# t0m1ab/alphazero

Measured on AMD Instinct MI355X. Metric: self-play games/sec (whole node), Othello 8x8 @100 sims/move, higher is better.
Workload: dtype f32; 1 GPU; BASELINE configs[1] literal: Othello 8x8, 4096 concurrent games/GPU, 100 sims/move, 1 MI355X; concurrent_games_per_gpu=4096, sims_per_move=100, parallelism=game-sharded x1, dense_layers=float32 fma chains on the f32-input MFMA

## Files before the change

### alphazero_amd/csrc/az_net.hip

```cpp
#include <math.h>
#include <stdlib.h>
#include <string.h>

#include <map>
#include <string>
#include <vector>

#include "az_device.h"
#include <hip/hip_ext.h>
#include "az_host.h"

typedef float f32x4 __attribute__((ext_vector_type(4)));
#define MFMA(a, b, c) __builtin_amdgcn_mfma_f32_16x16x4f32((a), (b), (c), 0, 0, 0)
typedef float f32x16 __attribute__((ext_vector_type(16)));
typedef float f32x2 __attribute__((ext_vector_type(2)));
#define MFMA32(a, b, c) __builtin_amdgcn_mfma_f32_32x32x2f32((a), (b), (c), 0, 0, 0)

#define NCH 32
#define PLANE_STRIDE(x) (((x) + 1) | 1)

#ifdef AZ_PROBE
__device__ unsigned long long az_probe_buf[8192 * 8];
#define STAMP(var) { __builtin_amdgcn_sched_barrier(0); var = __builtin_amdgcn_s_memtime(); asm volatile("s_waitcnt lgkmcnt(0)" ::: "memory"); __builtin_amdgcn_sched_barrier(0); }
#else
// ... 19 lines not shown
    const int m_lane = lane & 15, kq = lane >> 4;
    int abase[MT];
    unsigned vmask[MT];
#pragma unroll
    for (int mt = 0; mt < MT; ++mt) {
        int p = 16 * mt + m_lane;
        p = p < P_OUT ? p : P_OUT - 1;
        const int y = p / W_OUT, x = p % W_OUT;
        abase[mt] = kq * IN_PS + y * IN_W + x - PAD * (IN_W + 1);
        unsigned vm = 0;
#pragma unroll
        for (int t = 0; t < 9; ++t) {
            int iy = y + t / 3 - PAD, ix = x + t % 3 - PAD;
            vm |= (unsigned)(iy >= 0 && iy < H_OUT + 2 - 2 * PAD && ix >= 0 && ix < W_OUT + 2 - 2 * PAD) << t;
        }
        vmask[mt] = vm;
    }
    const float *wl = wf + 4 * lane;
    float bfr[2][16];
#pragma unroll
    for (int q = 0; q < 4; ++q) {
        const f32x4 v = *reinterpret_cast<const f32x4 *>(wl + q * 256);
        bfr[0][4 * q] = v[0]; bfr[0][4 * q + 1] = v[1]; bfr[0][4 * q + 2] = v[2]; bfr[0][4 * q + 3] = v[3];
    }
    const float bv0 = bias[m_lane], bv1 = bias[16 + m_lane];
#pragma unroll
    for (int mt = 0; mt < MT; ++mt) {
        acc[mt][0] = (f32x4){bv0, bv0, bv0, bv0};
        acc[mt][1] = (f32x4){bv1, bv1, bv1, bv1};
    }
    float ar[A_RING][MT];
#define CONV_LOAD(c, mt) in_lds[abase[mt] + ((c) / 8 / 3) * IN_W + ((c) / 8 % 3) + 4 * ((c) % 8) * IN_PS]
#pragma unroll
    for (int c = 0; c < A_RING; ++c)
#pragma unroll
        for (int mt = 0; mt < MT; ++mt) ar[c][mt] = CONV_LOAD(c, mt);
#pragma unroll
    for (int c = 0; c < 72; ++c) {
        const int tap = c / 8, j = c % 8;
        if (j == 0 && tap < 8) {
#pragma unroll
            for (int q = 0; q < 4; ++q) {
                const f32x4 v = *reinterpret_cast<const f32x4 *>(wl + ((tap + 1) * 4 + q) * 256);
                bfr[(tap + 1) & 1][4 * q] = v[0]; bfr[(tap + 1) & 1][4 * q + 1] = v[1];
                bfr[(tap + 1) & 1][4 * q + 2] = v[2]; bfr[(tap + 1) & 1][4 * q + 3] = v[3];
            }
        }
        float ac[MT];
#pragma unroll
        for (int mt = 0; mt < MT; ++mt) {
            float v = ar[c % A_RING][mt];
            if (PAD) v = ((vmask[mt] >> tap) & 1u) ? v : 0.0f;
            ac[mt] = v;
        }
        if (c + A_RING < 72) {
#pragma unroll
            for (int mt = 0; mt < MT; ++mt) ar[c % A_RING][mt] = CONV_LOAD(c + A_RING, mt);
        }
        __builtin_amdgcn_sched_barrier(0);
#pragma unroll
        for (int mt = 0; mt < MT; ++mt) {
            acc[mt][0] = MFMA(ac[mt], bfr[tap & 1][2 * j + 0], acc[mt][0]);
            acc[mt][1] = MFMA(ac[mt], bfr[tap & 1][2 * j + 1], acc[mt][1]);
        }
        __builtin_amdgcn_sched_barrier(0);
    }
#undef CONV_LOAD
}

template <int P_OUT, int OUT_PS, int MT>
AZ_D void store_relu_lds(float *out, int lane, const f32x4 (&acc)[MT][2]) {
#pragma unroll
    for (int mt = 0; mt < MT; ++mt)
#pragma unroll
        for (int nt = 0; nt < 2; ++nt)
#pragma unroll
            for (int r = 0; r < 4; ++r) {
                int m = 16 * mt + (lane >> 4) * 4 + r;
                float v = acc[mt][nt][r];
                if (m < P_OUT) out[(nt * 16 + (lane & 15)) * OUT_PS + m] = v > 0.0f ? v : 0.0f;
            }
}

template <int CH, int CW, int PS, int RING>
AZ_D void conv2_wino(float *act, const float4 *wu4, const float *__restrict__ bias, int lane) {
    constexpr int TW = (CW + 1) / 2, NTL = ((CH + 1) / 2) * TW, P1 = CH * CW;
    static_assert(NTL <= 16 && PS > P1, "one 16-row tile of 2x2 output tiles per board; a zero slot behind every plane");
    const int m = lane & 15, kq = lane >> 4;
    const int t = m < NTL ? m : NTL - 1;
    const int ty = t / TW, tx = t % TW;
    const float4 *ul = wu4 + lane;
    float cu[2][4][2], cw_[2][4][2];
    float yo[2][4][2][2];
#pragma unroll
    for (int p = 0; p < 2; ++p) {
        int off[12];
#pragma unroll
        for (int a = 0; a < 3; ++a)
#pragma unroll
            for (int b = 0; b < 4; ++b) {
                const int iy = 2 * ty - 1 + a + p, ix = 2 * tx - 1 + b;
                off[a * 4 + b] = kq * PS + ((iy >= 0 && iy < CH && ix >= 0 && ix < CW) ? iy * CW + ix : P1);
            }
        f32x4 acc[8][2];
#pragma unroll
        for (int f = 0; f < 8; ++f) { acc[f][0] = (f32x4){0.0f, 0.0f, 0.0f, 0.0f}; acc[f][1] = (f32x4){0.0f, 0.0f, 0.0f, 0.0f}; }
        float4 ub[RING][4];
#pragma unroll
        for (int jj = 0; jj < RING - 1; ++jj)
#pragma unroll
            for (int q = 0; q < 4; ++q) ub[jj][q] = ul[(size_t)((p * 8 + jj) * 4 + q) * 64];
        float d[12];
#pragma unroll
        for (int e = 0; e < 12; ++e) d[e] = act[off[e]];
#pragma unroll
        for (int j = 0; j < 8; ++j) {
            float dn[12];
            if (j + RING - 1 < 8) {
#pragma unroll
                for (int q = 0; q < 4; ++q) ub[(j + RING - 1) % RING][q] = ul[(size_t)((p * 8 + j + RING - 1) * 4 + q) * 64];
            }
            if (j + 1 < 8) {
#pragma unroll
                for (int e = 0; e < 12; ++e) dn[e] = act[off[e] + 4 * (j + 1) * PS];
            }
            float T[2][4], V[8];
#pragma unroll
            for (int b = 0; b < 4; ++b) {
                if (p == 0) { T[0][b] = d[b] - d[8 + b]; T[1][b] = d[4 + b] + d[8 + b]; }
                else { T[0][b] = d[4 + b] - d[b]; T[1][b] = d[b] - d[8 + b]; }
            }
#pragma unroll
            for (int i = 0; i < 2; ++i) {
                V[4 * i + 0] = T[i][0] - T[i][2]; V[4 * i + 1] = T[i][1] + T[i][2];
                V[4 * i + 2] = T[i][2] - T[i][1]; V[4 * i + 3] = T[i][1] - T[i][3];
            }
            __builtin_amdgcn_sched_barrier(0);
#pragma unroll
            for (int f = 0; f < 8; ++f) {
                const float4 u = ub[j % RING][f >> 1];
                acc[f][0] = MFMA(V[f], (f & 1) ? u.z : u.x, acc[f][0]);
                acc[f][1] = MFMA(V[f], (f & 1) ? u.w : u.y, acc[f][1]);
            }
#pragma unroll
            for (int f = 0; f < 8; ++f) { asm volatile("" : "+a"(acc[f][0])); asm volatile("" : "+a"(acc[f][1])); }
            __builtin_amdgcn_sched_barrier(0);
            if (j + 1 < 8) {
#pragma unroll
                for (int e = 0; e < 12; ++e) d[e] = dn[e];
            }
        }
#pragma unroll
        for (int nt = 0; nt < 2; ++nt)
#pragma unroll
            for (int r = 0; r < 4; ++r) {
                float R[2][2];
#pragma unroll
                for (int i = 0; i < 2; ++i) {
                    R[i][0] = (acc[4 * i + 0][nt][r] + acc[4 * i + 1][nt][r]) + acc[4 * i + 2][nt][r];
                    R[i][1] = (acc[4 * i + 1][nt][r] - acc[4 * i + 2][nt][r]) - acc[4 * i + 3][nt][r];
                }
#pragma unroll
                for (int c = 0; c < 2; ++c) {
                    if (p == 0) { cu[nt][r][c] = R[0][c] + R[1][c]; cw_[nt][r][c] = R[1][c]; }
                    else { yo[nt][r][0][c] = cu[nt][r][c] + R[0][c]; yo[nt][r][1][c] = (cw_[nt][r][c] - R[0][c]) - R[1][c]; }
                }
            }
    }
    LDS_FENCE();
#pragma unroll
    for (int nt = 0; nt < 2; ++nt) {
        const float bv = bias[nt * 16 + m];
#pragma unroll
        for (int r = 0; r < 4; ++r) {
            const int tt = 4 * kq + r, y0 = 2 * (tt / TW), x0 = 2 * (tt % TW);
#pragma unroll
            for (int i = 0; i < 2; ++i)
#pragma unroll
                for (int c = 0; c < 2; ++c) {
                    const float v = yo[nt][r][i][c] + bv;
                    if (tt < NTL && y0 + i < CH && x0 + c < CW) act[(nt * 16 + m) * PS + (y0 + i) * CW + x0 + c] = v > 0.0f ? v : 0.0f;
                }
        }
    }
}

template <int CH, int CW, int PS, int OFF1>
AZ_D void conv2_wino32(float *act, const float2 *u2, const float *__restrict__ bias, int lane) {
    constexpr int TW = (CW + 1) / 2, NTL = ((CH + 1) / 2) * TW, P1 = CH * CW;
    static_assert(2 * NTL <= 32 && PS > P1, "the tiles of two boards fill one 32-row MFMA tile");
    const int m = lane & 31, kk = lane >> 5;
    const int mc = m < 2 * NTL ? m : 2 * NTL - 1;
    const int bd = mc / NTL, t = mc % NTL, ty = t / TW, tx = t % TW;
    int off[16];
#pragma unroll
    for (int a = 0; a < 4; ++a)
#pragma unroll
        for (int b = 0; b < 4; ++b) {
            const int iy = 2 * ty - 1 + a, ix = 2 * tx - 1 + b;
            off[a * 4 + b] = bd * OFF1 + kk * PS + ((iy >= 0 && iy < CH && ix >= 0 && ix < CW) ? iy * CW + ix : P1);
        }
    f32x16 acc[16];
#pragma unroll
    for (int f = 0; f < 16; ++f)
#pragma unroll
        for (int i = 0; i < 16; ++i) acc[f][i] = 0.0f;
    const float2 *ul = u2 + lane;
    float d[16], V[2][16];
#define DP(e) ((f32x2){d[e], d[(e) + 1]})
#define WINO32_STAGE1(q, Tl, Th)                              \
    {                                                         \
        if ((q) == 0) Tl[0] = DP(0) - DP(8);                  \
        if ((q) == 1) Th[0] = DP(2) - DP(10);                 \
        if ((q) == 2) Tl[1] = DP(4) + DP(8);                  \
        if ((q) == 3) Th[1] = DP(6) + DP(10);                 \
        if ((q) == 4) Tl[2] = DP(8) - DP(4);                  \
        if ((q) == 5) Th[2] = DP(10) - DP(6);                 \
        if ((q) == 6) Tl[3] = DP(4) - DP(12);                 \
        if ((q) == 7) Th[3] = DP(6) - DP(14);                 \
    }
#define WINO32_STAGE2(i, c, Tl, Th, Vout)                                                          \
    {                                                                                              \
        if ((c) == 0) { const f32x2 v03 = Tl[i] - Th[i]; Vout[4 * (i) + 0] = v03.x; Vout[4 * (i) + 3] = v03.y; } \
        if ((c) == 1) Vout[4 * (i) + 1] = Tl[i].y + Th[i].x;                                       \
        if ((c) == 2) Vout[4 * (i) + 2] = Th[i].x - Tl[i].y;                                       \
    }
#define WINO32_FENCE() { __builtin_amdgcn_sched_barrier(0); asm volatile("" ::: "memory"); __builtin_amdgcn_sched_barrier(0); }
#pragma unroll
    for (int e = 0; e < 16; ++e) d[e] = act[off[e]];
    float2 ub[2][16];
#pragma unroll
    for (int f = 0; f < 16; ++f) ub[0][f] = ul[f * 64];
    {
        f32x2 Tl[4], Th[4];
#pragma unroll
        for (int q = 0; q < 8; ++q) WINO32_STAGE1(q, Tl, Th)
#pragma unroll
        for (int i = 0; i < 4; ++i)
#pragma unroll
            for (int c = 0; c < 3; ++c) WINO32_STAGE2(i, c, Tl, Th, V[0])
    }
#pragma unroll
    for (int e = 0; e < 16; ++e) d[e] = act[off[e] + 2 * PS];
    WINO32_FENCE()
    constexpr int DORD[16] = {0, 1, 8, 9, 2, 3, 10, 11, 4, 5, 6, 7, 12, 13, 14, 15};
#pragma unroll
    for (int j = 0; j < 16; ++j) {
        f32x2 Tl[4], Th[4];
#pragma unroll
        for (int g = 0; g < 16; ++g) {
            if (j + 1 < 16) {
                if (g < 8) WINO32_STAGE1(g, Tl, Th)
                if (g >= 2 && g < 14) WINO32_STAGE2((g - 2) / 3, (g - 2) % 3, Tl, Th, V[(j + 1) & 1])
            }
            if (j + 2 < 16 && g >= 8) {
                const int e0 = DORD[2 * (g - 8)], e1 = DORD[2 * (g - 8) + 1];
                d[e0] = act[off[e0] + 2 * (j + 2) * PS];
                d[e1] = act[off[e1] + 2 * (j + 2) * PS];
            }
            if (j % 2 == 0 && j + 2 < 16) ub[(j / 2 + 1) & 1][g] = ul[((j / 2 + 1) * 16 + g) * 64];
            WINO32_FENCE()
            acc[g] = MFMA32(V[j & 1][g], (j % 2 == 0) ? ub[(j / 2) & 1][g].x : ub[(j / 2) & 1][g].y, acc[g]);
            asm volatile("" : "+a"(acc[g]));
            WINO32_FENCE()
// ... 120 lines not shown
#pragma unroll
    for (int i = 0; i < NA; ++i)
        if (i < nu) {
#pragma unroll
            for (int q = 0; q < 4; ++q) {
                const int r = 16 * (par + 2 * i) + (lane >> 4) * 4 + q;
                const float v = acc[i][q];
                if (r < rows) out[(r / P_OUT) * OUT_BS + (nt * 16 + (lane & 15)) * OUT_CS + r % P_OUT] = v > 0.0f ? v : 0.0f;
            }
        }
}

template <int CH, int CW, bool WINO>
__global__ __launch_bounds__(256, 2) void k_trunk(const float *__restrict__ in, int B, const int *__restrict__ dyn_count, TrunkParams tp, float *__restrict__ feat) {
    using G = TrunkGeom<CH, CW>;
    if (dyn_count) { int c = *dyn_count; B = c < B ? c : B; }
    extern __shared__ __attribute__((aligned(16))) float smem[];
    const int wave = threadIdx.x >> 6, lane = threadIdx.x & 63;
    const int b = blockIdx.x * 4 + wave;
    if (b >= B) return;
    float *inp = smem + wave * G::WAVE_FLOATS;
    float *act = inp + G::INP;
    for (int i = lane; i < G::INP; i += 64) inp[i] = 0.0f;
    if (WINO && lane < NCH) act[lane * G::PS + G::P1] = 0.0f;
    LDS_FENCE();
    for (int p = lane; p < G::P1; p += 64) inp[(p / CW + 1) * G::PW + (p % CW) + 1] = in[(size_t)b * G::P1 + p];
    LDS_FENCE();
    {
        f32x4 acc[G::MT2][2];
        const int m_lane = lane & 15, kq = lane >> 4;
        const float bv0 = tp.b1[m_lane], bv1 = tp.b1[16 + m_lane];
#pragma unroll
        for (int s = 0; s < 3; ++s) {
            int tap = 4 * s + kq;
            tap = tap < 9 ? tap : 8;
            const int toff = (tap / 3) * G::PW + tap % 3;
            const float b0 = tp.w1f[(s * 2 + 0) * 64 + lane], b1 = tp.w1f[(s * 2 + 1) * 64 + lane];
#pragma unroll
            for (int mt = 0; mt < G::MT2; ++mt) {
                int p = 16 * mt + m_lane;
                p = p < G::P1 ? p : G::P1 - 1;
                const float a = inp[(p / CW) * G::PW + (p % CW) + toff];
                if (s == 0) { acc[mt][0] = (f32x4){bv0, bv0, bv0, bv0}; acc[mt][1] = (f32x4){bv1, bv1, bv1, bv1}; }
                acc[mt][0] = MFMA(a, b0, acc[mt][0]);
                acc[mt][1] = MFMA(a, b1, acc[mt][1]);
            }
        }
        store_relu_lds<G::P1, G::PS, G::MT2>(act, lane, acc);
    }
    LDS_FENCE();
    if constexpr (WINO) {
        conv2_wino<CH, CW, G::PS, 3>(act, reinterpret_cast<const float4 *>(tp.wu), tp.cb[0], lane);
    } else {
        f32x4 acc[G::MT2][2];
        conv_mfma<G::P1, CW, CH, CW, G::PS, 1, G::MT2>(act, tp.wq[0], tp.cb[0], lane, acc);
        LDS_FENCE();
        store_relu_lds<G::P1, G::PS, G::MT2>(act, lane, acc);
    }
    LDS_FENCE();
    {
        f32x4 acc[G::MT3][2];
        conv_mfma<G::P3, G::W3, G::H3, CW, G::PS, 0, G::MT3>(act, tp.wq[1], tp.cb[1], lane, acc);
        LDS_FENCE();
        store_relu_lds<G::P3, G::PS, G::MT3>(act, lane, acc);
    }
    LDS_FENCE();
    {
        f32x4 acc[G::MT4][2];
        conv_mfma<G::P4, G::W4, G::H4, G::W3, G::PS, 0, G::MT4>(act, tp.wq[2], tp.cb[2], lane, acc);
        float *fo = feat + (size_t)b * (NCH * G::P4);
#pragma unroll
        for (int mt = 0; mt < G::MT4; ++mt)
#pragma unroll
            for (int nt = 0; nt < 2; ++nt)
#pragma unroll
                for (int r = 0; r < 4; ++r) {
                    int m = 16 * mt + (lane >> 4) * 4 + r;
                    float v = acc[mt][nt][r];
                    if (m < G::P4) fo[(nt * 16 + (lane & 15)) * G::P4 + m] = v > 0.0f ? v : 0.0f;
                }
    }
}

template <int CH, int CW>
__global__ __launch_bounds__(256, 2) void k_trunk_quad(const float *__restrict__ in, int B, const int *__restrict__ dyn_count, TrunkParams tp, float *__restrict__ feat) {
    using G = TrunkGeom<CH, CW>;
    if (dyn_count) { int c = *dyn_count; B = c < B ? c : B; }
    extern __shared__ __attribute__((aligned(16))) float smem[];
    const int wave = threadIdx.x >> 6, lane = threadIdx.x & 63;
    const int b = blockIdx.x * 4 + wave;
    if ((int)blockIdx.x * 4 >= B) return;
    const bool has = b < B;
    const int nb = B - (int)blockIdx.x * 4 < 4 ? B - (int)blockIdx.x * 4 : 4;
    const int nt = wave >> 1, par = (wave & 1) ^ (__builtin_popcount(blockIdx.x) & 1);
    float *inp = smem + wave * G::WAVE_FLOATS;
    float *act = inp + G::INP;
    float *act0 = smem + G::INP;
    if (has) {
        for (int i = lane; i < G::INP; i += 64) inp[i] = 0.0f;
        if (lane < NCH) act[lane * G::PS + G::P1] = 0.0f;
        LDS_FENCE();
        for (int p = lane; p < G::P1; p += 64) inp[(p / CW + 1) * G::PW + (p % CW) + 1] = in[(size_t)b * G::P1 + p];
        LDS_FENCE();
    }
    if (has) {
        f32x4 acc[G::MT2][2];
        const int m_lane = lane & 15, kq = lane >> 4;
        const float bv0 = tp.b1[m_lane], bv1 = tp.b1[16 + m_lane];
#pragma unroll
        for (int s = 0; s < 3; ++s) {
            int tap = 4 * s + kq;
            tap = tap < 9 ? tap : 8;
            const int toff = (tap / 3) * G::PW + tap % 3;
            const float b0 = tp.w1f[(s * 2 + 0) * 64 + lane], b1 = tp.w1f[(s * 2 + 1) * 64 + lane];
#pragma unroll
            for (int mt = 0; mt < G::MT2; ++mt) {
                int p = 16 * mt + m_lane;
                p = p < G::P1 ? p : G::P1 - 1;
                const float a = inp[(p / CW) * G::PW + (p % CW) + toff];
                if (s == 0) { acc[mt][0] = (f32x4){bv0, bv0, bv0, bv0}; acc[mt][1] = (f32x4){bv1, bv1, bv1, bv1}; }
                acc[mt][0] = MFMA(a, b0, acc[mt][0]);
                acc[mt][1] = MFMA(a, b1, acc[mt][1]);
            }
        }
        store_relu_lds<G::P1, G::PS, G::MT2>(act, lane, acc);
        LDS_FENCE();
    }
    if (has) {
        conv2_wino<CH, CW, G::PS, 3>(act, reinterpret_cast<const float4 *>(tp.wu), tp.cb[0], lane);
        LDS_FENCE();
    }
    __syncthreads();
    {
        f32x4 acc[((4 * G::P3 + 15) / 16 + 1) / 2];
        const int nu = conv_quad_deal<G::P3, G::W3, CW, G::PS, G::WAVE_FLOATS>(act0, tp.wq[1], tp.cb[1], lane, nt, par, nb * G::P3, acc);
        __syncthreads();
        store_quad_relu<G::P3, G::PS, G::WAVE_FLOATS>(act0, lane, nt, par, nu, nb * G::P3, acc);
    }
    __syncthreads();
    {
        f32x4 acc[((4 * G::P4 + 15) / 16 + 1) / 2];
        const int nu = conv_quad_deal<G::P4, G::W4, G::W3, G::PS, G::WAVE_FLOATS>(act0, tp.wq[2], tp.cb[2], lane, nt, par, nb * G::P4, acc);
        store_quad_relu<G::P4, G::P4, NCH * G::P4>(feat + (size_t)blockIdx.x * 4 * (NCH * G::P4), lane, nt, par, nu, nb * G::P4, acc);
    }
}

template <int P_OUT, int W_OUT, int H_OUT, int IN_W, int IN_PS, int PAD>
AZ_D f32x4 conv_tile(const float *in_lds, const float *__restrict__ wf, const float *__restrict__ bias, int lane, int mt, int nt) {
    const int m_lane = lane & 15, kq = lane >> 4;
    int p = 16 * mt + m_lane;
    p = p < P_OUT ? p : P_OUT - 1;
    const int y = p / W_OUT, x = p % W_OUT;
    const int abase = kq * IN_PS + y * IN_W + x - PAD * (IN_W + 1);
    unsigned vmask = 0;
#pragma unroll
    for (int t = 0; t < 9; ++t) {
        int iy = y + t / 3 - PAD, ix = x + t % 3 - PAD;
        vmask |= (unsigned)(iy >= 0 && iy < H_OUT + 2 - 2 * PAD && ix >= 0 && ix < W_OUT + 2 - 2 * PAD) << t;
    }
    const float *wl = wf + 4 * lane;
    float bfr[2][8];
#define TILE_BLOAD(tap_, buf_)                                                             \
    _Pragma("unroll") for (int q = 0; q < 4; ++q) {                                        \
        const f32x4 v = *reinterpret_cast<const f32x4 *>(wl + ((tap_) * 4 + q) * 256);     \
        bfr[buf_][2 * q] = nt ? v[1] : v[0];                                               \
        bfr[buf_][2 * q + 1] = nt ? v[3] : v[2];                                           \
    }
    TILE_BLOAD(0, 0)
    const float bv = bias[16 * nt + m_lane];
    f32x4 acc = (f32x4){bv, bv, bv, bv};
    float ar[A_RING];
#define TILE_LOAD(c) in_lds[abase + ((c) / 8 / 3) * IN_W + ((c) / 8 % 3) + 4 * ((c) % 8) * IN_PS]
#pragma unroll
    for (int c = 0; c < A_RING; ++c) ar[c] = TILE_LOAD(c);
#pragma unroll
    for (int c = 0; c < 72; ++c) {
        const int tap = c / 8, j = c % 8;
        if (j == 0 && tap < 8) { TILE_BLOAD(tap + 1, (tap + 1) & 1) }
        float v = ar[c % A_RING];
        if (PAD) v = ((vmask >> tap) & 1u) ? v : 0.0f;
        if (c + A_RING < 72) ar[c % A_RING] = TILE_LOAD(c + A_RING);
        __builtin_amdgcn_sched_barrier(0);
        acc = MFMA(v, bfr[tap & 1][j], acc);
        __builtin_amdgcn_sched_barrier(0);
    }
#undef TILE_LOAD
#undef TILE_BLOAD
    return acc;
}

template <int P_OUT, int OUT_PS>
AZ_D void store_tile_relu_lds(float *out, int lane, const f32x4 &acc, int mt, int nt) {
#pragma unroll
    for (int r = 0; r < 4; ++r) {
        const int m = 16 * mt + (lane >> 4) * 4 + r;
        const float v = acc[r];
        if (m < P_OUT) out[(nt * 16 + (lane & 15)) * OUT_PS + m] = v > 0.0f ? v : 0.0f;
    }
}

template <int CH, int CW, int PS>
AZ_D void conv2_wino_pass(const float *act, const float4 *wu4, int lane, int nt, int p, float (&R)[4][2][2]) {
    constexpr int TW = (CW + 1) / 2, NTL = ((CH + 1) / 2) * TW, P1 = CH * CW, RING = 3;
    const int m = lane & 15, kq = lane >> 4;
    const int t = m < NTL ? m : NTL - 1;
    const int ty = t / TW, tx = t % TW;
    const float4 *ul = wu4 + lane + (size_t)p * 8 * 4 * 64;
    int off[12];
#pragma unroll
    for (int a = 0; a < 3; ++a)
#pragma unroll
        for (int b = 0; b < 4; ++b) {
// ... 2388 lines not shown
            AZ_TRY(fold_launch(n, FOLD_BIAS, (float *)n->tp.cb[l - 1], NCH, "", 0, cn + ".bias", NCH, bnn, NCH, 0, 0, 0, st));
            AZ_TRY(fold_launch(n, FOLD_WP, (float *)n->tp.wp[l - 1], 9 * 16 * 64, cn + ".weight", wn, "", 0, bnn, NCH, 0, 0, 0, st));
            AZ_TRY(fold_launch(n, FOLD_WQ, (float *)n->tp.wq[l - 1], 9 * 16 * 64, cn + ".weight", wn, "", 0, bnn, NCH, 0, 0, 0, st));
            if (l == 1) AZ_TRY(fold_launch(n, FOLD_WINO, (float *)n->tp.wu, 2 * 8 * 4 * 64 * 4, cn + ".weight", wn, "", 0, bnn, NCH, 0, 0, 0, st));
            if (l == 1) AZ_TRY(fold_launch(n, FOLD_WINO32, (float *)n->tp.wu32, 4 * 16 * 64 * 4, cn + ".weight", wn, "", 0, bnn, NCH, 0, 0, 0, st));
        }
    }
    AZ_TRY(fold_launch(n, FOLD_DENSE_T, n->fc1w, n->FIN * n->F1, "fc1.weight", (size_t)n->F1 * n->FIN, "", 0, "fc_bn1", n->F1, n->FIN, n->F1, 0, st));
    AZ_TRY(fold_launch(n, FOLD_BIAS, n->fc1b, n->F1, "", 0, "fc1.bias", n->F1, "fc_bn1", n->F1, 0, 0, 0, st));
    AZ_TRY(retile_q(n->fc1w, n->fc1wq, n->FIN, n->F1, st));
        AZ_TRY(quant_w(n, 1, st));
    AZ_TRY(fold_launch(n, FOLD_DENSE_T, n->fc2w, n->F1 * n->F2, "fc2.weight", (size_t)n->F2 * n->F1, "", 0, "fc_bn2", n->F2, n->F1, n->F2, 0, st));
    AZ_TRY(fold_launch(n, FOLD_BIAS, n->fc2b, n->F2, "", 0, "fc2.bias", n->F2, "fc_bn2", n->F2, 0, 0, 0, st));
    AZ_TRY(retile_q(n->fc2w, n->fc2wq, n->F1, n->F2, st));
        AZ_TRY(quant_w(n, 2, st));
    AZ_TRY(fold_launch(n, FOLD_HEADS_W, n->hw, n->F2 * n->NH, "fc_probs.weight", (size_t)n->A * n->F2, "fc_value.weight", n->F2, "", 0, n->F2, n->NH, n->A, st));
    AZ_TRY(fold_launch(n, FOLD_HEADS_B, n->hb, n->NH, "fc_probs.bias", n->A, "fc_value.bias", 1, "", 0, 0, n->NH, n->A, st));
    if (n->F2 % 16 == 0)
        AZ_TRY(fold_launch(n, FOLD_HEADS_WQ, n->hwq, n->F2 * n->NH, "fc_probs.weight", (size_t)n->A * n->F2, "fc_value.weight", n->F2, "", 0, n->F2, n->NH, n->A, st));
    AZ_HIP(hipGetLastError());
    n->committed = true;
    return AZ_OK;
}

static bool use_wino(int CH, int CW) {
    static int mode = -2;
    if (mode == -2) { const char *e = getenv("AZ_WINOGRAD"); mode = e ? atoi(e) : -1; }
    if (mode == 0) return false;
    return (CH == 8 && CW == 8) || (CH == 7 && CW == 6);
}

static thread_local hipEvent_t g_ev_start = nullptr, g_ev_stop = nullptr;
static thread_local int g_ev_used = 0;
#define AZ_LAUNCH_EV(ev0, ev1, kern, grid, block, lds, st, ...)                                                              \
    do {                                                                                                                     \
        if (g_ev_start) { hipExtLaunchKernelGGL(kern, grid, block, lds, st, ev0, ev1, 0, __VA_ARGS__); g_ev_used = 1; }      \
        else hipLaunchKernelGGL(kern, grid, block, lds, st, __VA_ARGS__);                                                    \
    } while (0)
#define AZ_LAUNCH(kern, grid, block, lds, st, ...) AZ_LAUNCH_EV(g_ev_start, g_ev_stop, kern, grid, block, lds, st, __VA_ARGS__)
static thread_local int g_ev_split = 0;
#define AZ_LAUNCH_FIRST(kern, grid, block, lds, st, ...)                                                                     \
    do { AZ_LAUNCH_EV(g_ev_start, nullptr, kern, grid, block, lds, st, __VA_ARGS__); g_ev_split = 1; } while (0)
#define AZ_LAUNCH_MAYBE_LAST(kern, grid, block, lds, st, ...)                                                                \
    do { AZ_LAUNCH_EV(g_ev_split ? nullptr : g_ev_start, g_ev_stop, kern, grid, block, lds, st, __VA_ARGS__); g_ev_split = 0; } while (0)

template <int CH, int CW, bool WINO>
static int launch_trunk2(az_net *n, const float *in, int B, const int *dyn, hipStream_t st) {
    using G = TrunkGeom<CH, CW>;
    constexpr int WPB = WINO ? 4 : 8;
    constexpr int lds_planes = 64 + WPB * 2 * G::WAVE_FLOATS * 4;
    constexpr int lds_bytes = lds_planes + ((WINO && lds_planes + 65536 <= 160 * 1024) ? 65536 : 0);
    static_assert(lds_bytes <= 160 * 1024, "k_trunk2 workgroup does not fit the CU's LDS");
    static int n_cu = 0;
    if (!n_cu) {
        hipDeviceProp_t pr;
        int dev = 0;
        AZ_HIP(hipGetDevice(&dev));
        AZ_HIP(hipGetDeviceProperties(&pr, dev));
        AZ_HIP(hipFuncSetAttribute(reinterpret_cast<const void *>(&k_trunk2<CH, CW, WPB, WINO>), hipFuncAttributeMaxDynamicSharedMemorySize, lds_bytes));
        n_cu = pr.multiProcessorCount;
    }
    const int pairs = (B + 1) / 2, want = (pairs + 3) / 4;
    AZ_LAUNCH((k_trunk2<CH, CW, WPB, WINO>), dim3(want < n_cu ? want : n_cu), dim3(64 * WPB), lds_bytes, st, in, B, dyn, n->tp, n->feat);
    return AZ_OK;
}

static thread_local int g_beside = 0;
static int beside_env(const char *name, int dflt) { const char *e = getenv(name); return e ? atoi(e) : dflt; }
static int beside_trunk2_min() { static int v = -2; if (v == -2) v = beside_env("AZ_BESIDE_TRUNK2_MIN", 4096); return v; }
static int beside_frag_max() { static int v = -2; if (v == -2) v = beside_env("AZ_BESIDE_FRAG_MAX", 1024); return v; }
static int beside_tile() { static int v = -2; if (v == -2) v = beside_env("AZ_BESIDE_TILE", 0); return v; }

static bool trunk_v1() { static int v = -1; if (v < 0) { const char *e = getenv("AZ_TRUNK_V1"); v = (e && atoi(e)) ? 1 : 0; } return v == 1; }

static int trunk_quad_env() { static int v = -2; if (v == -2) { const char *e = getenv("AZ_TRUNK_QUAD"); v = e ? (atoi(e) ? 1 : 0) : -1; } return v; }
template <int CH, int CW, bool WINO>
constexpr bool trunk_has_quad() { return WINO && ((CH == 8 && CW == 8) || (CH == 7 && CW == 6)); }
template <int CH, int CW>
static bool trunk_quad() {
    if (trunk_quad_env() >= 0) return trunk_quad_env() == 1;
    return (CH == 7 && CW == 6) || g_beside;
}

static int trunk_q_max() { static int v = -1; if (v < 0) { const char *e = getenv("AZ_TRUNK_Q_MAX"); v = e ? atoi(e) : 512; } return v; }

template <int CH, int CW, bool WINO>
static int launch_trunk(az_net *n, const float *in, int B, const int *dyn, hipStream_t st) {
    n->last_trunk_two_boards = (!trunk_v1() && B >= (g_beside ? beside_trunk2_min() : 4096)) ? 1 : 0;
    n->last_trunk_q = 0;
    if (n->last_trunk_two_boards) return launch_trunk2<CH, CW, WINO>(n, in, B, dyn, st);
    if (B <= trunk_q_max()) {
        n->last_trunk_q = 1;
        static int nw_env = -1;
        if (nw_env < 0) { const char *e = getenv("AZ_TRUNK_Q_WAVES"); nw_env = e ? atoi(e) : 0; }
        const int nw = nw_env ? nw_env : (B <= 256 ? 8 : 4);
        if (nw == 8) AZ_LAUNCH((k_trunk_q<CH, CW, WINO, 8>), dim3((unsigned)B), dim3(512), 0, st, in, B, dyn, n->tp, n->feat);
        else AZ_LAUNCH((k_trunk_q<CH, CW, WINO, 4>), dim3((unsigned)B), dim3(256), 0, st, in, B, dyn, n->tp, n->feat);
        return AZ_OK;
    }
    using G = TrunkGeom<CH, CW>;
    static bool attr_set = false;
    static int lds_bytes = G::LDS_BYTES;
    if (!attr_set) {
        const char *e = getenv("AZ_TRUNK_BLOCKS_PER_CU");
        int want = e ? atoi(e) : 3;
        if (want >= 1 && want <= 8 && 160 * 1024 / want > G::LDS_BYTES) lds_bytes = (160 * 1024 / want) & ~15;
        AZ_HIP(hipFuncSetAttribute(reinterpret_cast<const void *>(&k_trunk<CH, CW, WINO>), hipFuncAttributeMaxDynamicSharedMemorySize, lds_bytes));
        if constexpr (trunk_has_quad<CH, CW, WINO>())
            AZ_HIP(hipFuncSetAttribute(reinterpret_cast<const void *>(&k_trunk_quad<CH, CW>), hipFuncAttributeMaxDynamicSharedMemorySize, lds_bytes));
        attr_set = true;
    }
    if constexpr (trunk_has_quad<CH, CW, WINO>()) {
        if (trunk_quad<CH, CW>()) {
            AZ_LAUNCH((k_trunk_quad<CH, CW>), dim3((B + 3) / 4), dim3(256), lds_bytes, st, in, B, dyn, n->tp, n->feat);
            return AZ_OK;
        }
    }
    AZ_LAUNCH((k_trunk<CH, CW, WINO>), dim3((B + 3) / 4), dim3(256), lds_bytes, st, in, B, dyn, n->tp, n->feat);
    return AZ_OK;
}

template <int BM, int BN, int WM, int WN, int KT>
static int gemm_launch(const float *A, const float *Bw, const float *bias, float *C, int M, int N, int K, bool relu, const int *dyn, hipStream_t st) {
    constexpr int lds = gemm_lds_bytes<BM, BN>();
    static bool attr_set = false;
    if (!attr_set) {
        AZ_HIP(hipFuncSetAttribute(reinterpret_cast<const void *>(&k_gemm<BM, BN, WM, WN, true, KT>), hipFuncAttributeMaxDynamicSharedMemorySize, lds));
        AZ_HIP(hipFuncSetAttribute(reinterpret_cast<const void *>(&k_gemm<BM, BN, WM, WN, false, KT>), hipFuncAttributeMaxDynamicSharedMemorySize, lds));
        attr_set = true;
    }
    dim3 grid(N / BN, (M + BM - 1) / BM);
    if (relu) AZ_LAUNCH((k_gemm<BM, BN, WM, WN, true, KT>), grid, dim3(256), lds, st, A, Bw, bias, C, M, N, K, dyn);
    else AZ_LAUNCH((k_gemm<BM, BN, WM, WN, false, KT>), grid, dim3(256), lds, st, A, Bw, bias, C, M, N, K, dyn);
    return AZ_OK;
}

template <int BM, int BN, int WM, int WN>
static int gemm_go(const float *A, const float *Bw, const float *bias, float *C, int M, int N, int K, bool relu, const int *dyn, hipStream_t st) {
    switch (K) {
        case 1024: return gemm_launch<BM, BN, WM, WN, 32>(A, Bw, bias, C, M, N, K, relu, dyn, st);
        case 512: return gemm_launch<BM, BN, WM, WN, 16>(A, Bw, bias, C, M, N, K, relu, dyn, st);
        case 192: return gemm_launch<BM, BN, WM, WN, 6>(A, Bw, bias, C, M, N, K, relu, dyn, st);
        case 128: return gemm_launch<BM, BN, WM, WN, 4>(A, Bw, bias, C, M, N, K, relu, dyn, st);
        case 64: return gemm_launch<BM, BN, WM, WN, 2>(A, Bw, bias, C, M, N, K, relu, dyn, st);
        default: return gemm_launch<BM, BN, WM, WN, 0>(A, Bw, bias, C, M, N, K, relu, dyn, st);
    }
}

template <int TM, int TN>
static int solo_t_launch(const float *A, const float *Bw, const float *bias, float *C, int M, int N, int K, bool relu, const int *dyn, hipStream_t st) {
    constexpr int BM = 64 * TM, BN = 64 * TN, lds = 4 * (2 * BM * 33 + 2 * 32 * BN);
    static bool attr_set = false;
    if (!attr_set) {
        AZ_HIP(hipFuncSetAttribute(reinterpret_cast<const void *>(&k_gemm_solo_t<true, TM, TN>), hipFuncAttributeMaxDynamicSharedMemorySize, lds));
        AZ_HIP(hipFuncSetAttribute(reinterpret_cast<const void *>(&k_gemm_solo_t<false, TM, TN>), hipFuncAttributeMaxDynamicSharedMemorySize, lds));
        attr_set = true;
    }
    dim3 grid(N / BN, (M + BM - 1) / BM);
    if (relu) AZ_LAUNCH((k_gemm_solo_t<true, TM, TN>), grid, dim3(256), lds, st, A, Bw, bias, C, M, N, K, dyn);
    else AZ_LAUNCH((k_gemm_solo_t<false, TM, TN>), grid, dim3(256), lds, st, A, Bw, bias, C, M, N, K, dyn);
    return AZ_OK;
}

enum GemmKind { GK_SMALL, GK_FRAG, GK_SOLO, GK_SOLO_T, GK_TILED };
static int gemm_solo_env() { static int solo = -2; if (solo == -2) { const char *e = getenv("AZ_GEMM_SOLO"); solo = e ? atoi(e) : -1; } return solo; }
static int frag_max_rows(int K) {
    static int v = -2;
    if (v == -2) { const char *e = getenv("AZ_DENSE_FRAG_MAX"); v = e ? atoi(e) : -1; }
    return v >= 0 ? v : (K >= 1024 ? 2048 : 1024);
}
static GemmKind gemm_kind(int M, int N, int K, bool have_q = true) {
    const int fmax = (g_beside && beside_frag_max() < frag_max_rows(K)) ? beside_frag_max() : frag_max_rows(K);
    if (have_q && M <= fmax && frag_shape(N, K)) return GK_FRAG;
    if (M <= (K >= 1024 ? 256 : 128) && K % 32 == 0) return GK_SMALL;
    const int solo = gemm_solo_env();
    const long long tiles = (long long)((M + 255) / 256) * (N / 256);
    if (solo != 0 && N % 256 == 0 && (solo == 1 || tiles >= 256)) return GK_SOLO;
    if (solo != 0 && solo != 1 && N % 128 == 0) {
        const long long t128 = (long long)((M + 127) / 128) * (N / 128);
        if (solo == 2 || (solo < 0 && t128 >= 512)) return GK_SOLO_T;
    }
    return GK_TILED;
}

static int frag_go(const float *A, const float *Bq, const float *bias, float *C, int M, int N, int K, bool relu, const int *dyn, hipStream_t st) {
    constexpr int NT = 4;
    const int lds = 4 * 16 * (K + 4);
    static int attr_lds = 0;
    if (lds > attr_lds) {
        AZ_HIP(hipFuncSetAttribute(reinterpret_cast<const void *>(&k_dense_frag<true, NT>), hipFuncAttributeMaxDynamicSharedMemorySize, lds));
        AZ_HIP(hipFuncSetAttribute(reinterpret_cast<const void *>(&k_dense_frag<false, NT>), hipFuncAttributeMaxDynamicSharedMemorySize, lds));
        attr_lds = lds;
    }
    dim3 grid((unsigned)(N / (16 * NT)), (unsigned)((M + 15) / 16));
    if (relu) AZ_LAUNCH((k_dense_frag<true, NT>), grid, dim3(64 * NT), lds, st, A, Bq, bias, C, M, N, K, dyn);
    else AZ_LAUNCH((k_dense_frag<false, NT>), grid, dim3(64 * NT), lds, st, A, Bq, bias, C, M, N, K, dyn);
    return AZ_OK;
// ... 424 lines not shown
```

Baseline: 4432 games/s.

## Split Winograd conv into four single-row passes to raise trunk-quad occupancy

Adds a four-pass variant of the 2x2 Winograd convolution that handles one frequency row per pass instead of two. This halves the live accumulators and input-transform registers, and compiler barriers pin the live ranges. k_trunk_quad becomes templated on a form that selects the pass count, ring depth and launch bounds (3 or 4 waves per EU). For 8x8 boards the LDS request is left at the minimum rather than padded to 3 blocks per CU. The cost is more passes, with extra weight and activation loads and more scheduling barriers, traded for higher occupancy.

```diff
diff --git a/alphazero_amd/csrc/az_net.hip b/alphazero_amd/csrc/az_net.hip
--- a/alphazero_amd/csrc/az_net.hip
+++ b/alphazero_amd/csrc/az_net.hip
@@ -125,18 +125,100 @@
             }
 }
 
-template <int CH, int CW, int PS, int RING>
+template <int CH, int CW, int PS, int RING, int NP = 2>
 AZ_D void conv2_wino(float *act, const float4 *wu4, const float *__restrict__ bias, int lane) {
     constexpr int TW = (CW + 1) / 2, NTL = ((CH + 1) / 2) * TW, P1 = CH * CW;
     static_assert(NTL <= 16 && PS > P1, "one 16-row tile of 2x2 output tiles per board; a zero slot behind every plane");
+    static_assert(NP == 2 || NP == 4, "two passes of two frequency rows or four passes of one");
     const int m = lane & 15, kq = lane >> 4;
     const int t = m < NTL ? m : NTL - 1;
     const int ty = t / TW, tx = t % TW;
     const float4 *ul = wu4 + lane;
     float cu[2][4][2], cw_[2][4][2];
     float yo[2][4][2][2];
-#pragma unroll
-    for (int p = 0; p < 2; ++p) {
+    if constexpr (NP == 4) {
+#pragma unroll
+        for (int i = 0; i < 4; ++i) {
+            constexpr int RA[4] = {0, 1, 2, 1}, RB[4] = {2, 2, 1, 3};
+            int off[8], li = lane;
+            asm volatile("" : "+v"(li));
+            const int mi = li & 15, kqi = li >> 4, ti = mi < NTL ? mi : NTL - 1, tyi = ti / TW, txi = ti % TW;
+#pragma unroll
+            for (int a = 0; a < 2; ++a)
+#pragma unroll
+                for (int b = 0; b < 4; ++b) {
+                    const int iy = 2 * tyi - 1 + (a ? RB[i] : RA[i]), ix = 2 * txi - 1 + b;
+                    off[a * 4 + b] = kqi * PS + ((iy >= 0 && iy < CH && ix >= 0 && ix < CW) ? iy * CW + ix : P1);
+                }
+            f32x4 acc[4][2];
+#pragma unroll
+            for (int f = 0; f < 4; ++f) { acc[f][0] = (f32x4){0.0f, 0.0f, 0.0f, 0.0f}; acc[f][1] = (f32x4){0.0f, 0.0f, 0.0f, 0.0f}; }
+            const float4 *up = ul + (size_t)((i >> 1) * 32 + 2 * (i & 1)) * 64;
+            float4 ub[RING][2];
+#pragma unroll
+            for (int jj = 0; jj < RING - 1; ++jj)
+#pragma unroll
+                for (int q = 0; q < 2; ++q) ub[jj][q] = up[(size_t)(jj * 4 + q) * 64];
+            float d[8];
+#pragma unroll
+            for (int e = 0; e < 8; ++e) d[e] = act[off[e]];
+#pragma unroll
+            for (int j = 0; j < 8; ++j) {
+                float dn[8];
+                if (j + RING - 1 < 8) {
+#pragma unroll
+                    for (int q = 0; q < 2; ++q) ub[(j + RING - 1) % RING][q] = up[(size_t)((j + RING - 1) * 4 + q) * 64];
+                }
+                if (j + 1 < 8) {
+#pragma unroll
+                    for (int e = 0; e < 8; ++e) dn[e] = act[off[e] + 4 * (j + 1) * PS];
+                }
+                float T[4], V[4];
+#pragma unroll
+                for (int b = 0; b < 4; ++b) T[b] = (i == 1) ? d[b] + d[4 + b] : d[b] - d[4 + b];
+                V[0] = T[0] - T[2]; V[1] = T[1] + T[2]; V[2] = T[2] - T[1]; V[3] = T[1] - T[3];
+                __builtin_amdgcn_sched_barrier(0);
+#pragma unroll
+                for (int f = 0; f < 4; ++f) {
+                    const float4 u = ub[j % RING][f >> 1];
+                    acc[f][0] = MFMA(V[f], (f & 1) ? u.z : u.x, acc[f][0]);
+                    acc[f][1] = MFMA(V[f], (f & 1) ? u.w : u.y, acc[f][1]);
+                }
+                __builtin_amdgcn_sched_barrier(0);
+                if (j + 1 < 8) {
+#pragma unroll
+                    for (int e = 0; e < 8; ++e) d[e] = dn[e];
+                }
+            }
+#pragma unroll
+            for (int nt = 0; nt < 2; ++nt)
+#pragma unroll
+                for (int r = 0; r < 4; ++r) {
+                    const float R0 = (acc[0][nt][r] + acc[1][nt][r]) + acc[2][nt][r];
+                    const float R1 = (acc[1][nt][r] - acc[2][nt][r]) - acc[3][nt][r];
+                    const float R[2] = {R0, R1};
+#pragma unroll
+                    for (int c = 0; c < 2; ++c) {
+                        if (i == 0) yo[nt][r][0][c] = R[c];
+                        else if (i == 1) { yo[nt][r][0][c] = yo[nt][r][0][c] + R[c]; yo[nt][r][1][c] = R[c]; }
+                        else if (i == 2) { yo[nt][r][0][c] = yo[nt][r][0][c] + R[c]; yo[nt][r][1][c] = yo[nt][r][1][c] - R[c]; }
+                        else yo[nt][r][1][c] = yo[nt][r][1][c] - R[c];
+                    }
+                }
+#pragma unroll
+            for (int nt = 0; nt < 2; ++nt)
+#pragma unroll
+                for (int r = 0; r < 4; ++r)
+#pragma unroll
+                    for (int c = 0; c < 2; ++c) {
+                        if (i < 3) asm volatile("" : "+v"(yo[nt][r][0][c]));
+                        if (i > 0) asm volatile("" : "+v"(yo[nt][r][1][c]));
+                    }
+            __builtin_amdgcn_sched_barrier(0);
+        }
+    }
+#pragma unroll
+    for (int p = 0; p < (NP == 4 ? 0 : 2); ++p) {
         int off[12];
 #pragma unroll
         for (int a = 0; a < 3; ++a)
@@ -211,18 +293,21 @@
             }
     }
     LDS_FENCE();
+    int le = lane;
+    if constexpr (NP == 4) asm volatile("" : "+v"(le));
+    const int kqe = le >> 4, me = le & 15;
 #pragma unroll
     for (int nt = 0; nt < 2; ++nt) {
-        const float bv = bias[nt * 16 + m];
+        const float bv = bias[nt * 16 + me];
 #pragma unroll
         for (int r = 0; r < 4; ++r) {
-            const int tt = 4 * kq + r, y0 = 2 * (tt / TW), x0 = 2 * (tt % TW);
+            const int tt = 4 * kqe + r, y0 = 2 * (tt / TW), x0 = 2 * (tt % TW);
 #pragma unroll
             for (int i = 0; i < 2; ++i)
 #pragma unroll
                 for (int c = 0; c < 2; ++c) {
                     const float v = yo[nt][r][i][c] + bv;
-                    if (tt < NTL && y0 + i < CH && x0 + c < CW) act[(nt * 16 + m) * PS + (y0 + i) * CW + x0 + c] = v > 0.0f ? v : 0.0f;
+                    if (tt < NTL && y0 + i < CH && x0 + c < CW) act[(nt * 16 + me) * PS + (y0 + i) * CW + x0 + c] = v > 0.0f ? v : 0.0f;
                 }
         }
     }
@@ -509,8 +594,8 @@
     }
 }
 
-template <int CH, int CW>
-__global__ __launch_bounds__(256, 2) void k_trunk_quad(const float *__restrict__ in, int B, const int *__restrict__ dyn_count, TrunkParams tp, float *__restrict__ feat) {
+template <int CH, int CW, int FORM>
+__global__ __launch_bounds__(256, FORM == 1 ? 4 : FORM == 2 ? 3 : 2) void k_trunk_quad(const float *__restrict__ in, int B, const int *__restrict__ dyn_count, TrunkParams tp, float *__restrict__ feat) {
     using G = TrunkGeom<CH, CW>;
     if (dyn_count) { int c = *dyn_count; B = c < B ? c : B; }
     extern __shared__ __attribute__((aligned(16))) float smem[];
@@ -554,7 +639,7 @@
         LDS_FENCE();
     }
     if (has) {
-        conv2_wino<CH, CW, G::PS, 3>(act, reinterpret_cast<const float4 *>(tp.wu), tp.cb[0], lane);
+        conv2_wino<CH, CW, G::PS, FORM == 1 ? 2 : 3, FORM ? 4 : 2>(act, reinterpret_cast<const float4 *>(tp.wu), tp.cb[0], lane);
         LDS_FENCE();
     }
     __syncthreads();
@@ -3109,6 +3194,12 @@
     return (CH == 7 && CW == 6) || g_beside;
 }
 
+static int trunk_quad_form(int CH) {
+    static int v = -2;
+    if (v == -2) { const char *e = getenv("AZ_TRUNK_QUAD_FORM"); v = e ? atoi(e) : -1; }
+    return (v >= 0 && v <= 2) ? v : (CH == 8 ? 2 : 1);
+}
+
 static int trunk_q_max() { static int v = -1; if (v < 0) { const char *e = getenv("AZ_TRUNK_Q_MAX"); v = e ? atoi(e) : 512; } return v; }
 
 template <int CH, int CW, bool WINO>
@@ -3127,19 +3218,26 @@
     }
     using G = TrunkGeom<CH, CW>;
     static bool attr_set = false;
-    static int lds_bytes = G::LDS_BYTES;
+    static int lds_bytes = G::LDS_BYTES, lds_lean = G::LDS_BYTES;
     if (!attr_set) {
         const char *e = getenv("AZ_TRUNK_BLOCKS_PER_CU");
-        int want = e ? atoi(e) : 3;
+        const int want = e ? atoi(e) : 3, want_lean = e ? atoi(e) : ((CH == 8 && CW == 8) ? 0 : 3);
         if (want >= 1 && want <= 8 && 160 * 1024 / want > G::LDS_BYTES) lds_bytes = (160 * 1024 / want) & ~15;
+        if (want_lean >= 1 && want_lean <= 8 && 160 * 1024 / want_lean > G::LDS_BYTES) lds_lean = (160 * 1024 / want_lean) & ~15;
         AZ_HIP(hipFuncSetAttribute(reinterpret_cast<const void *>(&k_trunk<CH, CW, WINO>), hipFuncAttributeMaxDynamicSharedMemorySize, lds_bytes));
-        if constexpr (trunk_has_quad<CH, CW, WINO>())
-            AZ_HIP(hipFuncSetAttribute(reinterpret_cast<const void *>(&k_trunk_quad<CH, CW>), hipFuncAttributeMaxDynamicSharedMemorySize, lds_bytes));
+        if constexpr (trunk_has_quad<CH, CW, WINO>()) {
+            AZ_HIP(hipFuncSetAttribute(reinterpret_cast<const void *>(&k_trunk_quad<CH, CW, 0>), hipFuncAttributeMaxDynamicSharedMemorySize, lds_bytes));
+            AZ_HIP(hipFuncSetAttribute(reinterpret_cast<const void *>(&k_trunk_quad<CH, CW, 1>), hipFuncAttributeMaxDynamicSharedMemorySize, lds_lean));
+            AZ_HIP(hipFuncSetAttribute(reinterpret_cast<const void *>(&k_trunk_quad<CH, CW, 2>), hipFuncAttributeMaxDynamicSharedMemorySize, lds_lean));
+        }
         attr_set = true;
     }
     if constexpr (trunk_has_quad<CH, CW, WINO>()) {
         if (trunk_quad<CH, CW>()) {
-            AZ_LAUNCH((k_trunk_quad<CH, CW>), dim3((B + 3) / 4), dim3(256), lds_bytes, st, in, B, dyn, n->tp, n->feat);
+            const int form = trunk_quad_form(CH);
+            if (form == 1) AZ_LAUNCH((k_trunk_quad<CH, CW, 1>), dim3((B + 3) / 4), dim3(256), lds_lean, st, in, B, dyn, n->tp, n->feat);
+            else if (form == 2) AZ_LAUNCH((k_trunk_quad<CH, CW, 2>), dim3((B + 3) / 4), dim3(256), lds_lean, st, in, B, dyn, n->tp, n->feat);
+            else AZ_LAUNCH((k_trunk_quad<CH, CW, 0>), dim3((B + 3) / 4), dim3(256), lds_bytes, st, in, B, dyn, n->tp, n->feat);
             return AZ_OK;
         }
     }
```

Result: faster. 4523 games/s (median of 6 runs) (+2.1%).
